# ChainSafe/lumenos

Measured on AMD Instinct MI355X. Metric: prove_eval_seconds_16384x4096, lower is better.
Workload: dtype u64; 1 GPU; Encode+Commit+InnerProduct(r,b)+QueryCols 16384x4096 LogN=14 L=12 K=2 rhoInv=2 queries=309; parallelism=1 GPU: the whole job resident in HBM

## Files before the change

### lumenos_amd/csrc/lm_keyswitch.hip

```cpp
#include <cstdlib>
#include <cstring>

#include "lm_ks_dev.h"

__host__ __device__ __forceinline__ size_t ks_ext_at(uint32_t b, uint32_t d, uint32_t t, uint32_t B, uint32_t beta) {
    return ((size_t)t * B + b) * beta + d;
}
__host__ __device__ __forceinline__ size_t ks_u_at(uint32_t pw, uint32_t t, uint32_t B, uint32_t L, uint32_t K) {
    return t < L ? (size_t)t * 2 * B + pw : (size_t)L * 2 * B + (size_t)pw * K + (t - L);
}
__host__ __device__ __forceinline__ size_t ks_key_at(uint32_t d, uint32_t w, uint32_t t, uint32_t beta) {
    return ((size_t)t * beta + d) * 2 + w;
}

static uint32_t ks_batch(const lumen_ctx *ctx) { return ctx->tune.ks_batch; }

__device__ __forceinline__ void mul128(u64 a, u64 b, u64 &lo, u64 &hi) {
    const u32 a0 = (u32)a, a1 = (u32)(a >> 32), b0 = (u32)b, b1 = (u32)(b >> 32);
    const u64 p0 = (u64)a0 * b0;
    const u64 p1 = lm_keep((u64)a0 * b1 + (p0 >> 32));
    const u64 p2 = lm_keep((u64)a1 * b0 + (u32)p1);
    hi = (u64)a1 * b1 + (p1 >> 32) + (p2 >> 32);
    lo = (p2 << 32) | (u32)p0;
}
// ... 42 lines not shown
            pack_pair(a, b, m0, m1, M, hi, lo);
            if (e) hv.y = hi, lv.y = lo;
            else hv.x = hi, lv.x = lo;
        }
        *reinterpret_cast<ulonglong2 *>(y0) = hv;
        *reinterpret_cast<ulonglong2 *>(y0 + N) = lv;
    }
}

template <int LOGN>
__global__ __launch_bounds__(lm_max_threads(LOGN)) void k_intt_pack(const u64 *__restrict__ acc, u64 *coef, uint32_t B,
                                                                  uint32_t L, uint32_t nf, lm_mods mods,
                                                                  lm_ninv_t yscale, const tw_t *__restrict__ tw_all) {
    extern __shared__ __attribute__((aligned(16))) u64 sm[];
    constexpr uint32_t N = 1u << LOGN;
    const uint32_t tid = threadIdx.x, nthreads = blockDim.x;
    if (blockIdx.x >= B * nf) {
        const uint32_t k = blockIdx.x - B * nf, l = 2 * nf + k / B, b = k % B;
        const u64 *p = acc + (((size_t)b * 2 + 1) * L + l) * N;
        u64 *o = coef + ((size_t)b * L + l) * N;
        const lm_qc q = lm_make_qc(mods.m[l]);
        const tw_t sc = yscale.t[l];
        auto ld = [&](uint32_t i0, u64 *v, int count) { lm_load_run(p, i0, v, count); };
        auto st = [&](uint32_t i, u64 v) { o[i] = lm_shoup_cs(v, sc, q.q, q.nq); };
        lm_ntt_inverse<LOGN>(sm, tw_all + (size_t)l * N, q, tid, nthreads, ld, st);
        return;
    }
    const uint32_t d = blockIdx.x / B, b = blockIdx.x % B;
    const uint32_t l0 = 2 * d, l1 = l0 + 1;
    const u64 *c1 = acc + ((size_t)b * 2 + 1) * L * N;
    u64 *o0 = coef + ((size_t)b * L + l0) * N;
    const lm_qc q0 = lm_make_qc(mods.m[l0]);
    const tw_t s0 = yscale.t[l0];
    {
        const u64 *p = c1 + (size_t)l0 * N;
        auto ld = [&](uint32_t i0, u64 *v, int count) { lm_load_run(p, i0, v, count); };
        auto st = [&](uint32_t i, u64 v) { o0[i] = lm_shoup_cs(v, s0, q0.q, q0.nq); };
        lm_ntt_inverse<LOGN>(sm, tw_all + (size_t)l0 * N, q0, tid, nthreads, ld, st);
    }
    __syncthreads();
    {
        const lm_qc q1 = lm_make_qc(mods.m[l1]);
        const tw_t s1 = yscale.t[l1];
        const u64 *p = c1 + (size_t)l1 * N;
        u64 Ml, Mh;
        mul128(q0.q, q1.q, Ml, Mh);
        auto uni = [](u64 x) {
            return (u64)(uint32_t)__builtin_amdgcn_readfirstlane((int)(uint32_t)x) |
                   (u64)(uint32_t)__builtin_amdgcn_readfirstlane((int)(uint32_t)(x >> 32)) << 32;
        };
        const u128 M = ((u128)uni(Mh) << 64) | uni(Ml);
        auto ld = [&](uint32_t i0, u64 *v, int count) { lm_load_run(p, i0, v, count); };
        constexpr int R_LAST = lm_pass_r(LOGN, 0), LOG_T0 = LOGN - R_LAST;
        constexpr int PF = (1 << R_LAST) * 5 / 8;
        struct pack_t {
            u64 *o0;
            const lm_qc &q0, &q1;
            tw_t s1;
            u128 M;
            u64 y0[PF];
            __device__ __forceinline__ void pre(uint32_t w) {
#pragma unroll
                for (int k = 0; k < PF; k++) y0[k] = o0[w + ((uint32_t)k << LOG_T0)];
            }
            __device__ __forceinline__ void operator()(uint32_t i, u64 v, int k) {
                const u64 y1 = lm_shoup_cs(v, s1, q1.q, q1.nq);
                uint32_t j = i;
                asm volatile("" : "+v"(j));
                const u64 a = k < PF ? y0[k < PF ? k : 0] : o0[j];
                u64 hi, lo;
                pack_pair(a, y1, q0.q, q1.q, M, hi, lo);
                o0[j] = hi, o0[j + N] = lo;
                if (k >= PF && (k & 1)) asm volatile("" ::: "memory");
            }
        } st{o0, q0, q1, s1, M, {}};
        uint32_t tid1 = tid;
        asm volatile("" : "+v"(tid1));
        lm_ntt_inverse<LOGN>(sm, tw_all + (size_t)l1 * N, q1, tid1, nthreads, ld, st);
    }
}

struct pt_consts_t {
    u64 c[LM_MAX_LIMBS];
};
__global__ void k_pt_prepare(const u64 *__restrict__ pt, u64 *__restrict__ ptM, uint32_t logN, uint32_t nl,
                             lm_mods mods, pt_consts_t pc) {
    const size_t total = (size_t)nl << logN;
    for (size_t i = (size_t)blockIdx.x * blockDim.x + threadIdx.x; i < total; i += (size_t)gridDim.x * blockDim.x) {
        const uint32_t limb = (uint32_t)(i >> logN);
        u64 lo, hi;
        mul128(pt[i], pc.c[limb], lo, hi);
        ptM[i] = lm_mont_reduce(lo, hi, mods.m[limb].q, mods.m[limb].qneg);
    }
}
__global__ void k_mul_plain(const u64 *__restrict__ ct, u64 *__restrict__ out, const u64 *__restrict__ ptM,
                            size_t words, uint32_t logN, uint32_t nl, lm_mods mods) {
    const size_t stride = (size_t)gridDim.x * blockDim.x;
    const size_t N = (size_t)1 << logN;
    for (size_t i = (size_t)blockIdx.x * blockDim.x + threadIdx.x; i < words; i += stride) {
        const uint32_t limb = (uint32_t)((i >> logN) % nl);
        const size_t k = i & (N - 1);
        u64 lo, hi;
        mul128(ct[i], ptM[(size_t)limb * N + k], lo, hi);
        out[i] = lm_mont_reduce(lo, hi, mods.m[limb].q, mods.m[limb].qneg);
    }
}

template <int LOGN>
__global__ __launch_bounds__(lm_fwdw_threads(LOGN), lm_fwdw_waves(LOGN)) void k_modup_ntt(const u64 *__restrict__ coef, const u64 *__restrict__ acc,
                                                    u64 *__restrict__ ext, const bx_t *__restrict__ bx,
                                                    uint32_t B, uint32_t L, uint32_t K, uint32_t beta,
                                                    const uint32_t *__restrict__ work, lm_mods mods,
                                                    const tw_t *__restrict__ tw_all) {
    extern __shared__ __attribute__((aligned(16))) u64 sm[];
    constexpr uint32_t N = 1u << LOGN;
    const uint32_t tid = threadIdx.x, nthreads = blockDim.x, LK = L + K;
    const uint32_t wk = work[blockIdx.x];
    const uint32_t b = wk & 0xFFFF, d = (wk >> 16) & 0xFF, t = wk >> 24;
    const bx_t c = bx[d * LK + t];
    u64 *o = ext + ks_ext_at(b, d, t, B, beta) * N;
    const lm_qc qc = lm_make_qc(mods.m[t]);
    const u64 *s0 = coef + ((size_t)b * L + d * K) * N;
    const u64 *s1 = c.ns == 2 ? s0 + N : s0;
    auto ld = [&](uint32_t i) { return bx_apply(c, s0[i], s1[i], qc); };
    auto out = [&](uint32_t j, u64 v0, u64 v1) {
        ulonglong2 y;
        y.x = v0, y.y = v1;
        *reinterpret_cast<ulonglong2 *>(o + j) = y;
    };
    if constexpr (LOGN == 14) {
        (void)nthreads;
        lm_w14_runs st{sm};
        auto after = [&](uint32_t i0, uint32_t) { lm_w14_linear_out(sm, tid, i0, out); };
        lm_ntt_forward_w14(sm, tw_all + (size_t)t * N, qc, tid, ld, st, after);
    } else {
        lm_lds_runs st{sm};
        auto after = [&](uint32_t, uint32_t) { lm_linear_out<LOGN>(sm, tid, out); };
        lm_ntt_forward<LOGN>(sm, tw_all + (size_t)t * N, qc, tid, nthreads, ld, st, after);
    }
}

#ifndef LM_MAC_COLS
#define LM_MAC_COLS 4
#endif
#ifndef LM_MAC_VEC
#define LM_MAC_VEC 1
#endif
#ifndef LM_MAC_PREFETCH
#define LM_MAC_PREFETCH 1
#endif
template <int VEC>
struct mac_vec;
template <>
struct mac_vec<1> {
    u64 v[1];
    static __device__ __forceinline__ mac_vec load(const u64 *p) { return mac_vec{{*p}}; }
    static __device__ __forceinline__ mac_vec load_once(const u64 *p) { return mac_vec{{__builtin_nontemporal_load(p)}}; }
    __device__ __forceinline__ void store(u64 *p) const { *p = v[0]; }
};
template <>
struct mac_vec<2> {
    u64 v[2];
    static __device__ __forceinline__ mac_vec load(const u64 *p) {
        const ulonglong2 a = *reinterpret_cast<const ulonglong2 *>(p);
        return mac_vec{{a.x, a.y}};
    }
    static __device__ __forceinline__ mac_vec load_once(const u64 *p) {
        return mac_vec{{__builtin_nontemporal_load(p), __builtin_nontemporal_load(p + 1)}};
    }
    __device__ __forceinline__ void store(u64 *p) const {
        ulonglong2 a;
        a.x = v[0], a.y = v[1];
        *reinterpret_cast<ulonglong2 *>(p) = a;
    }
};
struct mac_acc {
    u64 a0, a1, a3;
    u32 c0, c1;
    __device__ __forceinline__ void clear() { a0 = a1 = a3 = 0, c0 = c1 = 0; }
    __device__ __forceinline__ void value(u64 &lo, u64 &hi) const {
        lo = a0 + (a1 << 32);
        hi = a3 + c0 + (a1 >> 32) + ((u64)c1 << 32) + (lo < a0 ? 1 : 0);
    }
};
__device__ __forceinline__ void mac2(mac_acc &p, mac_acc &q, u64 x, u64 k0, u64 k1) {
    const u32 x0 = (u32)x, x1 = (u32)(x >> 32);
#if LM_ASM_SHOUP
    asm("v_mad_u64_u32 %[pa0], s[98:99], %[x0], %[k00], %[pa0]\n\t"
        "v_mad_u64_u32 %[qa0], s[90:91], %[x0], %[k10], %[qa0]\n\t"
        "v_mad_u64_u32 %[pa1], s[94:95], %[x0], %[k01], %[pa1]\n\t"
        "v_addc_co_u32_e64 %[pc0], s[96:97], %[pc0], 0, s[98:99]\n\t"
        "v_mad_u64_u32 %[qa1], s[92:93], %[x0], %[k11], %[qa1]\n\t"
        "v_addc_co_u32_e64 %[qc0], s[96:97], %[qc0], 0, s[90:91]\n\t"
        "v_mad_u64_u32 %[pa3], s[96:97], %[x1], %[k01], %[pa3]\n\t"
        "v_addc_co_u32_e64 %[pc1], s[96:97], %[pc1], 0, s[94:95]\n\t"
        "v_mad_u64_u32 %[pa1], s[98:99], %[x1], %[k00], %[pa1]\n\t"
        "v_addc_co_u32_e64 %[qc1], s[96:97], %[qc1], 0, s[92:93]\n\t"
        "v_mad_u64_u32 %[qa1], s[90:91], %[x1], %[k10], %[qa1]\n\t"
        "v_mad_u64_u32 %[qa3], s[96:97], %[x1], %[k11], %[qa3]\n\t"
        "v_addc_co_u32_e64 %[pc1], s[96:97], %[pc1], 0, s[98:99]\n\t"
        "v_addc_co_u32_e64 %[qc1], s[96:97], %[qc1], 0, s[90:91]"
        : [pa0] "+v"(p.a0), [pa1] "+v"(p.a1), [pa3] "+v"(p.a3), [pc0] "+v"(p.c0), [pc1] "+v"(p.c1),
          [qa0] "+v"(q.a0), [qa1] "+v"(q.a1), [qa3] "+v"(q.a3), [qc0] "+v"(q.c0), [qc1] "+v"(q.c1)
        : [x0] "v"(x0), [x1] "v"(x1), [k00] "v"((u32)k0), [k01] "v"((u32)(k0 >> 32)), [k10] "v"((u32)k1),
          [k11] "v"((u32)(k1 >> 32))
        : "s92", "s93", "s94", "s95", "s96", "s97", "s98", "s99", "s90", "s91");
#else
    auto one = [&](mac_acc &r, u64 k) {
        const u32 k0w = (u32)k, k1w = (u32)(k >> 32);
        u64 t = r.a0 + (u64)x0 * k0w;
        r.c0 += t < r.a0, r.a0 = t;
        t = r.a1 + (u64)x0 * k1w;
        r.c1 += t < r.a1, r.a1 = t;
        t = r.a1 + (u64)x1 * k0w;
        r.c1 += t < r.a1, r.a1 = t;
        r.a3 += (u64)x1 * k1w;
    };
    one(p, k0);
    one(q, k1);
#endif
}

__global__ __launch_bounds__(256) void k_ks_mac(const u64 *__restrict__ ext, const u64 *__restrict__ acc,
                                                const u64 *__restrict__ key, u64 *__restrict__ u, uint32_t B,
                                                uint32_t L, uint32_t K, uint32_t beta, uint32_t logN,
                                                lm_mods mods) {
    typedef mac_vec<LM_MAC_VEC> vec;
    const uint32_t N = 1u << logN, LK = L + K;
    const uint32_t G = (B + LM_MAC_COLS - 1) / LM_MAC_COLS, per_limb = N / (256 * LM_MAC_VEC) ? N / (256 * LM_MAC_VEC) : 1;
    const uint32_t slices = per_limb * LK;
    uint32_t slice, z;
    if (slices % 8 == 0) {
        const uint32_t xcd = blockIdx.x & 7, j = blockIdx.x >> 3;
        z = j % G;
        slice = (j / G) * 8 + xcd;
    } else {
        z = blockIdx.x % G;
        slice = blockIdx.x / G;
    }
    const uint32_t i = ((slice % per_limb) * 256 + threadIdx.x) * LM_MAC_VEC;
    const uint32_t t = LK - 1 - slice / per_limb;
    const uint32_t b0 = z * LM_MAC_COLS;
    if (i >= N) return;
    const mod_t md = mods.m[t];
    const uint32_t own = t < L ? t / K : 0xFFFFFFFFu;
    mac_acc a0[LM_MAC_COLS][LM_MAC_VEC], a1[LM_MAC_COLS][LM_MAC_VEC];
#pragma unroll
    for (int c = 0; c < LM_MAC_COLS; c++)
#pragma unroll
        for (int e = 0; e < LM_MAC_VEC; e++) a0[c][e].clear(), a1[c][e].clear();
    struct digit_t {
        vec k0, k1, x[LM_MAC_COLS];
    };
    auto fetch = [&](uint32_t d) {
        digit_t g;
        g.k0 = vec::load(key + ks_key_at(d, 0, t, beta) * N + i);
        g.k1 = vec::load(key + ks_key_at(d, 1, t, beta) * N + i);
#pragma unroll
        for (int c = 0; c < LM_MAC_COLS; c++) {
            const uint32_t bc = b0 + c < B ? b0 + c : B - 1;
            g.x[c] = d == own ? vec::load(acc + ((size_t)(bc * 2 + 1) * L + t) * N + i)
                              : vec::load_once(ext + ks_ext_at(bc, d, t, B, beta) * N + i);
        }
        return g;
    };
    constexpr int PF = LM_MAC_PREFETCH;
    digit_t q[PF + 1];
#pragma unroll
    for (int j = 0; j < PF; j++)
        if ((uint32_t)j < beta) q[j] = fetch(j);
    for (uint32_t d0 = 0; d0 < beta; d0 += PF + 1) {
#pragma unroll
        for (int j = 0; j <= PF; j++) {
            const uint32_t d = d0 + j;
            if (d < beta) {
                if (d + PF < beta) q[(j + PF) % (PF + 1)] = fetch(d + PF);
#pragma unroll
                for (int c = 0; c < LM_MAC_COLS; c++)
#pragma unroll
                    for (int e = 0; e < LM_MAC_VEC; e++) mac2(a0[c][e], a1[c][e], q[j].x[c].v[e], q[j].k0.v[e], q[j].k1.v[e]);
            }
        }
    }
#pragma unroll
    for (int c = 0; c < LM_MAC_COLS; c++) {
        if (b0 + c < B) {
            u64 *o = u + ks_u_at((b0 + c) * 2, t, B, L, K) * N + i, *o1 = u + ks_u_at((b0 + c) * 2 + 1, t, B, L, K) * N + i;
            vec r0, r1;
#pragma unroll
            for (int e = 0; e < LM_MAC_VEC; e++) {
                u64 lo, hi;
                a0[c][e].value(lo, hi);
                r0.v[e] = lm_mont_reduce_wide(lo, hi, md.q, md.qneg, md.qinv64, beta);
                a1[c][e].value(lo, hi);
                r1.v[e] = lm_mont_reduce_wide(lo, hi, md.q, md.qneg, md.qinv64, beta);
            }
            r0.store(o);
            r1.store(o1);
        }
    }
}

template <int LOGN>
__global__ __launch_bounds__(lm_max_threads(LOGN)) void k_moddown_ntt(const u64 *__restrict__ u, const u64 *__restrict__ acc_in,
                                                     u64 *__restrict__ acc_out, const bx_t *__restrict__ bxp,
                                                     const tw_t *__restrict__ pinv,
                                                     const uint32_t *__restrict__ index,
                                                     const uint32_t *__restrict__ inv_index,
                                                     const uint32_t *__restrict__ work, uint32_t B,
                                                     uint32_t L, uint32_t K, lm_mods mods,
                                                     const tw_t *__restrict__ tw_all) {
    extern __shared__ __attribute__((aligned(16))) u64 sm[];
    constexpr uint32_t N = 1u << LOGN;
    const uint32_t tid = threadIdx.x, nthreads = blockDim.x;
    const uint32_t wk = work[blockIdx.x];
    const uint32_t pw = wk & 0xFFFF;
    const uint32_t t = wk >> 16;
    const uint32_t w = pw & 1;
    const bx_t c = bxp[t];
    const lm_qc qc = lm_make_qc(mods.m[t]);
    const u64 *up0 = u + ks_u_at(pw, L, B, L, K) * N;
    const u64 *up1 = c.ns == 2 ? up0 + N : up0;
    const u64 *uq = u + ks_u_at(pw, t, B, L, K) * N;
    const u64 *ain = acc_in + ((size_t)pw * L + t) * N;
    u64 *aout = acc_out + ((size_t)pw * L + t) * N;
    tw_t pi = pinv[t];
    pi.w = qc.q - pi.w, pi.wp = ~pi.wp;
    auto ld = [&](uint32_t i) { return bx_apply(c, up0[i], up1[i], qc); };
    constexpr int RUN = lm_fwd_run<LOGN>();
    static_assert(RUN <= 8, "lm_load_run moves at most 8 coefficients");
    struct storer_t {
        const u64 *uq, *ain;
        u64 *sm;
        const lm_qc &qc;
        tw_t pi;
        uint32_t w;
        u64 uv[RUN], cv[RUN];
        __device__ __forceinline__ void pre(uint32_t i0) {
            lm_load_run(uq, i0, uv, RUN);
            if (w == 0) lm_load_run(ain, i0, cv, RUN);
        }
        __device__ __forceinline__ void operator()(uint32_t i0, const u64 *v, int count) {
#pragma unroll
            for (int k = 0; k < RUN; k++)
                if (k < count) {
                    const u64 add = w == 0 ? uv[k] + cv[k] : uv[k];
                    sm[LM_PAD(i0 + k)] = lm_shoup3<true>(v[k], pi.w, pi.wp, qc.nq, add);
                }
        }
    } st{uq, ain, sm, qc, pi, w, {}, {}};
    constexpr uint32_t NW = lm_nthreads(LOGN) / 64, BLK = N / NW, IT = BLK / 128;
    const uint32_t wave = tid >> 6, lane = tid & 63;
    const uint32_t jb = NW > 1 ? (uint32_t)__builtin_amdgcn_readfirstlane((int)(inv_index[wave * BLK] / BLK)) : 0u;
    auto after = [&](uint32_t, uint32_t) {
        uint2 p[IT];
        ulonglong2 x[IT];
#pragma unroll
        for (uint32_t k = 0; k < IT; k++) {
            const uint32_t j = jb * BLK + 2 * lane + k * 128;
            p[k] = *reinterpret_cast<const uint2 *>(index + j);
            x[k] = *reinterpret_cast<const ulonglong2 *>(ain + j);
        }
        lm_wave_sync();
#pragma unroll
        for (uint32_t k = 0; k < IT; k++) {
            const uint32_t j = jb * BLK + 2 * lane + k * 128;
            ulonglong2 y;
            y.x = lm_csub(lm_csub(x[k].x + sm[LM_PAD(p[k].x)], 4 * qc.q), 2 * qc.q);
            y.y = lm_csub(lm_csub(x[k].y + sm[LM_PAD(p[k].y)], 4 * qc.q), 2 * qc.q);
            *reinterpret_cast<ulonglong2 *>(aout + j) = y;
        }
    };
    lm_ntt_forward<LOGN>(sm, tw_all + (size_t)t * N, qc, tid, nthreads, ld, st, after);
}

__global__ __launch_bounds__(256) void k_acc_canon(u64 *__restrict__ acc, size_t pairs, uint32_t logN, uint32_t L, lm_mods mods) {
    const size_t stride = (size_t)gridDim.x * blockDim.x;
    for (size_t g = (size_t)blockIdx.x * blockDim.x + threadIdx.x; g < pairs; g += stride) {
        const u64 q = mods.m[(uint32_t)((g >> (logN - 1)) % L)].q;
        ulonglong2 v = *reinterpret_cast<ulonglong2 *>(acc + 2 * g);
        v.x = lm_csub(v.x, q), v.y = lm_csub(v.y, q);
        *reinterpret_cast<ulonglong2 *>(acc + 2 * g) = v;
    }
}

namespace {

int acc_canon(lumen_ctx *ctx, u64 *acc, size_t words, uint32_t L) {
    if (!words) return 0;
    hipLaunchKernelGGL(k_acc_canon, dim3(2048), dim3(256), 0, ctx->stream, acc, words / 2, ctx->logN, L, ctx->mods);
    LM_HIP(ctx, hipGetLastError());
    return 0;
}

struct KsTables {
    bx_t *d_bx = nullptr;
    bx_t *d_bxp = nullptr;
    tw_t *d_pinv = nullptr;
    uint32_t beta = 0;
    lm_ninv_t yscale;
    std::vector<uint16_t> pairs;
    std::map<uint32_t, uint32_t *> d_work;
    std::map<uint32_t, uint32_t *> d_work_down;
    ~KsTables() {
        for (auto &kv : d_work) hipFree(kv.second);
        for (auto &kv : d_work_down) hipFree(kv.second);
        hipFree(d_bx);
        hipFree(d_bxp);
        hipFree(d_pinv);
    }
};

bx_t make_bx(const uint64_t *src, uint32_t ns, uint64_t t) {
    bx_t c;
    memset(&c, 0, sizeof(c));
    c.ns = ns;
    uint64_t m_mod_t = 1;
    for (uint32_t a = 0; a < ns; a++) m_mod_t = h_mulmod(m_mod_t, src[a] % t, t);
    c.b57 = h_tw((1ull << LM_W_SPLIT) % t, t);
    c.c_t = (t - h_mulmod(2 % t, m_mod_t, t)) % t;
    return c;
}

uint64_t hat_inv(const uint64_t *src, uint32_t ns, uint32_t a) {
    uint64_t h = 1;
    for (uint32_t b = 0; b < ns; b++)
        if (b != a) h = h_mulmod(h, src[b] % src[a], src[a]);
    return h_invmod(h, src[a]);
}

int get_tables(lumen_ctx *ctx, KsTables **out) {
    LM_SHARED_LOCK(ctx);
    auto it = ctx->ext.find("ks_tables");
    if (it != ctx->ext.end()) {
        *out = static_cast<KsTables *>(it->second.get());
        return 0;
    }
    const uint32_t L = ctx->L, K = ctx->K, LK = L + K;
    LM_CHECK(ctx, K >= 1 && K <= 2, "key switching supports 1 or 2 special primes (have %u)", K);
    auto sp = std::make_shared<KsTables>();
    KsTables &tb = *sp;
    tb.beta = (L + K - 1) / K;
    std::vector<bx_t> bx((size_t)tb.beta * LK);
    for (uint32_t d = 0; d < tb.beta; d++) {
        const uint32_t lo = d * K, hi = std::min(lo + K, L), ns = hi - lo;
        for (uint32_t t = 0; t < LK; t++) {
            bx_t c = make_bx(ctx->mod + lo, ns, ctx->mod[t]);
            c.own = (t >= lo && t < hi) ? 1 : 0;
            bx[(size_t)d * LK + t] = c;
        }
    }
    for (uint32_t i = 0; i < LM_MAX_LIMBS; i++) tb.yscale.t[i] = ctx->ninv[i < LK ? i : 0];
    for (uint32_t d = 0; d < tb.beta; d++) {
        const uint32_t lo = d * K, hi = std::min(lo + K, L), ns = hi - lo;
        for (uint32_t a = 0; a < ns; a++) {
            const uint64_t m = ctx->mod[lo + a];
            tb.yscale.t[lo + a] = h_tw(h_mulmod(ctx->ninv[lo + a].w, hat_inv(ctx->mod + lo, ns, a), m), m);
        }
    }
    for (uint32_t a = 0; a < K; a++) {
        const uint64_t m = ctx->mod[L + a];
        tb.yscale.t[L + a] = h_tw(h_mulmod(ctx->ninv[L + a].w, hat_inv(ctx->mod + L, K, a), m), m);
    }
    std::vector<bx_t> bxp(L);
    std::vector<tw_t> pinv(L);
    for (uint32_t t = 0; t < L; t++) {
        bxp[t] = make_bx(ctx->mod + L, K, ctx->mod[t]);
        uint64_t q = ctx->mod[t], P = 1;
        for (uint32_t a = 0; a < K; a++) P = h_mulmod(P, ctx->mod[L + a] % q, q);
        pinv[t] = h_tw(h_invmod(P, q), q);
    }
    std::vector<uint16_t> pairs;
    for (uint32_t t = 0; t < LK; t++)
        for (uint32_t d = 0; d < tb.beta; d++)
            if (!bx[(size_t)d * LK + t].own) pairs.push_back((uint16_t)(d | (t << 8)));
    tb.pairs = pairs;
    LM_HIP(ctx, hipMalloc((void **)&tb.d_bx, bx.size() * sizeof(bx_t)));
    LM_HIP(ctx, hipMalloc((void **)&tb.d_bxp, bxp.size() * sizeof(bx_t)));
    LM_HIP(ctx, hipMalloc((void **)&tb.d_pinv, pinv.size() * sizeof(tw_t)));
    LM_HIP(ctx, hipMemcpy(tb.d_bx, bx.data(), bx.size() * sizeof(bx_t), hipMemcpyHostToDevice));
    LM_HIP(ctx, hipMemcpy(tb.d_bxp, bxp.data(), bxp.size() * sizeof(bx_t), hipMemcpyHostToDevice));
    LM_HIP(ctx, hipMemcpy(tb.d_pinv, pinv.data(), pinv.size() * sizeof(tw_t), hipMemcpyHostToDevice));
    ctx->ext["ks_tables"] = sp;
    *out = sp.get();
    return 0;
}

}

int lm_ks_tables_view(lumen_ctx *ctx, lm_ks_view *out) {
    KsTables *tb = nullptr;
    if (int rc = get_tables(ctx, &tb)) return rc;
    out->d_bxp = tb->d_bxp;
    out->d_pinv = tb->d_pinv;
    out->yscale = &tb->yscale;
    return 0;
}

int lm_launch_pack_v(lumen_ctx *ctx, u64 *y, size_t poly_stride, uint32_t npoly, uint32_t ngroups,
                     uint32_t group_limbs, uint32_t first_mod, uint32_t nlimbs_total) {
    hipLaunchKernelGGL(k_pack_v, dim3(2048), dim3(256), 0, ctx->stream, y, poly_stride, npoly, ngroups, group_limbs,
                       first_mod, nlimbs_total, ctx->logN, ctx->mods);
    LM_HIP(ctx, hipGetLastError());
    return 0;
}

namespace {

struct KsScratch {
    u64 *coef, *ext, *u, *acc2;
};

static int modup_work_list(lumen_ctx *ctx, KsTables *tb, uint32_t B, const uint32_t **out) {
    const uint32_t LM_MODUP_TGROUP = ctx->tune.modup_tgroup;
    LM_SHARED_LOCK(ctx);
    LM_CHECK(ctx, B >= 1 && B <= 65535 && tb->beta <= 255 && ctx->L + ctx->K <= 255,
             "key-switch batch of %u columns (beta %u) does not fit the packed work list", B, tb->beta);
    const uint32_t cache_key = B | (LM_MODUP_TGROUP << 16);
    auto it = tb->d_work.find(cache_key);
    if (it != tb->d_work.end()) {
        *out = it->second;
        return 0;
    }
    const uint32_t LK = ctx->L + ctx->K, beta = tb->beta;
    std::vector<std::vector<uint8_t>> need(beta);
    for (uint16_t pr : tb->pairs) need[pr & 0xFF].push_back((uint8_t)(pr >> 8));
    std::vector<std::vector<uint32_t>> lists(8);
    for (uint32_t x = 0; x < 8; x++)
        for (uint32_t t0 = 0; t0 < LK; t0 += LM_MODUP_TGROUP)
            for (uint32_t b = x; b < B; b += 8)
                for (uint32_t d = 0; d < beta; d++)
                    for (uint8_t t : need[d])
                        if (t >= t0 && t < t0 + LM_MODUP_TGROUP) lists[x].push_back(b | (d << 16) | ((uint32_t)t << 24));
    std::vector<uint32_t> order;
    order.reserve((size_t)B * tb->pairs.size());
    std::vector<size_t> pos(8, 0);
    for (bool any = true; any;) {
        any = false;
        for (uint32_t x = 0; x < 8; x++)
            if (pos[x] < lists[x].size()) {
                order.push_back(lists[x][pos[x]++]);
                any = true;
            }
    }
    LM_CHECK(ctx, order.size() == (size_t)B * tb->pairs.size(), "extension work list is inconsistent");
    uint32_t *d = nullptr;
    LM_HIP(ctx, hipMalloc((void **)&d, order.size() * sizeof(uint32_t)));
    LM_HIP(ctx, hipMemcpy(d, order.data(), order.size() * sizeof(uint32_t), hipMemcpyHostToDevice));
    tb->d_work[cache_key] = d;
    *out = d;
    return 0;
}

static int moddown_work_list(lumen_ctx *ctx, KsTables *tb, uint32_t B, const uint32_t **out) {
    const uint32_t LM_MODDOWN_TGROUP = ctx->tune.moddown_tgroup;
    LM_SHARED_LOCK(ctx);
    LM_CHECK(ctx, B >= 1 && 2 * (uint64_t)B <= 65535, "key-switch batch of %u columns does not fit the packed work list", B);
    const uint32_t cache_key = B | (LM_MODDOWN_TGROUP << 17);
    auto it = tb->d_work_down.find(cache_key);
    if (it != tb->d_work_down.end()) {
        *out = it->second;
        return 0;
    }
    const uint32_t L = ctx->L;
    std::vector<std::vector<uint32_t>> lists(8);
    for (uint32_t x = 0; x < 8; x++)
        for (uint32_t t0 = 0; t0 < L; t0 += LM_MODDOWN_TGROUP)
            for (uint32_t pw = x; pw < 2 * B; pw += 8)
                for (uint32_t t = t0; t < std::min<uint32_t>(t0 + LM_MODDOWN_TGROUP, L); t++) lists[x].push_back(pw | (t << 16));
    std::vector<uint32_t> order;
    order.reserve((size_t)2 * B * L);
    std::vector<size_t> pos(8, 0);
    for (bool any = true; any;) {
        any = false;
        for (uint32_t x = 0; x < 8; x++)
            if (pos[x] < lists[x].size()) {
                order.push_back(lists[x][pos[x]++]);
                any = true;
            }
    }
    LM_CHECK(ctx, order.size() == (size_t)2 * B * L, "ModDown work list is inconsistent");
    uint32_t *d = nullptr;
    LM_HIP(ctx, hipMalloc((void **)&d, order.size() * sizeof(uint32_t)));
    LM_HIP(ctx, hipMemcpy(d, order.data(), order.size() * sizeof(uint32_t), hipMemcpyHostToDevice));
    tb->d_work_down[cache_key] = d;
    *out = d;
    return 0;
}

static uint32_t ks_lanes(const lumen_ctx *ctx) {
    return ctx->tune.ks_lanes ? ctx->tune.ks_lanes : (ctx->logN <= 13 ? 2 : 1);
}
template <int LOGN>
static uint32_t intt_pack_slots(lumen_ctx *ctx) {
    static const uint32_t v = [&] {
        hipDeviceProp_t prop;
        int per_cu = 0;
        if (hipGetDeviceProperties(&prop, ctx->device) != hipSuccess) return 256u;
        (void)hipFuncSetAttribute(reinterpret_cast<const void *>(&k_intt_pack<LOGN>),
                                  hipFuncAttributeMaxDynamicSharedMemorySize, 160 * 1024);
        if (hipOccupancyMaxActiveBlocksPerMultiprocessor(&per_cu, k_intt_pack<LOGN>, lm_nthreads(LOGN),
                                                         lm_lds_for(1u << LOGN)) != hipSuccess || per_cu < 1) {
            per_cu = (int)std::max<size_t>(1, std::min<size_t>(160 * 1024 / lm_lds_for(1u << LOGN), 2048 / lm_nthreads(LOGN)));
        }
        (void)hipGetLastError();
        if (ctx->tune.debug)
            fprintf(stderr, "[lumenos_hip] k_intt_pack<%d>: %d workgroup(s) per CU, %d CUs\n", LOGN, per_cu,
                    prop.multiProcessorCount);
        return (uint32_t)prop.multiProcessorCount * (uint32_t)per_cu;
    }();
    return v;
}
static uint32_t ks_fused_digits(lumen_ctx *ctx, uint32_t B, uint32_t L) {
    const long forced = ctx->tune.ks_fused_digits;
    const uint32_t pairs = L / 2;
    if (forced >= 0) return std::min<uint32_t>((uint32_t)forced, pairs);
    uint32_t slots = 0;
    switch (ctx->logN) {
#define LM_CASE(n) \
    case n: slots = intt_pack_slots<n>(ctx); break;
        LM_FOR_EACH_LOGN(LM_CASE)
#undef LM_CASE
    default: return 0;
    }
    for (uint32_t nf = pairs; nf >= 1; nf--)
        if (((uint64_t)B * nf) % slots == 0) return nf;
    return 0;
}

struct LaneGuard {
    lumen_ctx *ctx;
    hipStream_t saved;
    LaneGuard(lumen_ctx *c, int lane) : ctx(c), saved(c->stream) {
        if (lane) ctx->stream = ctx->stream2;
    }
    ~LaneGuard() { ctx->stream = saved; }
};

int rotate_accumulate(lumen_ctx *ctx, const u64 *acc, u64 *acc_out, uint32_t B, const lm_galois_key &gk,
                      KsTables *tb, const KsScratch &s) {
    const uint32_t N = ctx->N, L = ctx->L, K = ctx->K, LK = L + K, beta = tb->beta;
    const size_t lds = lm_fwd_lds(ctx->logN);
    const uint32_t threads = lm_fwd_threads(ctx->logN);
    const uint32_t nf = K == 2 ? ks_fused_digits(ctx, B, L) : 0;
    if (nf) {
        const size_t lds_i = lm_inv_lds(ctx->logN);
        const uint32_t grid = B * nf + B * (L - 2 * nf);
        lm_prof_scope ps(ctx, "ks_intt_c1", (uint64_t)B * L);
        switch (ctx->logN) {
#define LM_CASE(n)                                                                                              \
    case n:                                                                                                     \
        LM_LDS_ATTR(ctx, k_intt_pack<n>, lds_i);                                                                \
        hipLaunchKernelGGL(k_intt_pack<n>, dim3(grid), dim3(lm_inv_threads(ctx->logN)), lds_i, ctx->stream, acc, \
                           s.coef, B, L, nf, ctx->mods, tb->yscale, ctx->d_tw_inv);                             \
        break;
            LM_FOR_EACH_LOGN(LM_CASE)
#undef LM_CASE
        default:
            return lm_fail(ctx, "ring degree 2^%u has no kernel instantiation", ctx->logN);
        }
        LM_HIP(ctx, hipGetLastError());
    } else {
        if (int rc = lm_launch_ntt_strided(ctx, acc + (size_t)L * N, (size_t)2 * L * N, s.coef, (size_t)L * N, B,
                                           lm_map_q(L), true, "ks_intt_c1", &tb->yscale))
            return rc;
    }
    if (K == 2 && nf < beta) {
        lm_prof_scope ps(ctx, "ks_pack_v", (uint64_t)B);
        hipLaunchKernelGGL(k_pack_v, dim3(2048), dim3(256), 0, ctx->stream, s.coef + (size_t)2 * nf * N, (size_t)L * N,
                           B, beta - nf, K, 2 * nf, L - 2 * nf, ctx->logN, ctx->mods);
        LM_HIP(ctx, hipGetLastError());
    }
    {
        const uint64_t nb = (uint64_t)B * tb->pairs.size();
        const uint32_t *work = nullptr;
        if (int rc = modup_work_list(ctx, tb, B, &work)) return rc;
        lm_prof_scope ps(ctx, "ks_modup_ntt", nb);
        const lm_geom gm = lm_fwdw_geom(ctx->logN);
        switch (ctx->logN) {
#define LM_CASE(n)                                                                                            \
    case n:                                                                                                   \
        LM_LDS_ATTR(ctx, k_modup_ntt<n>, gm.lds);                                                             \
        hipLaunchKernelGGL(k_modup_ntt<n>, dim3((uint32_t)nb), dim3(gm.threads), gm.lds, ctx->stream, s.coef, acc, \
                           s.ext, tb->d_bx, B, L, K, beta, work, ctx->mods, ctx->d_tw_fwd);                   \
        break;
            LM_FOR_EACH_LOGN(LM_CASE)
#undef LM_CASE
        default:
            return lm_fail(ctx, "ring degree 2^%u has no kernel instantiation", ctx->logN);
        }
        LM_HIP(ctx, hipGetLastError());
    }
    {
        lm_prof_scope ps(ctx, "ks_mac", (uint64_t)B);
        dim3 grid(((N / LM_MAC_VEC + 255) / 256) * LK * ((B + LM_MAC_COLS - 1) / LM_MAC_COLS));
        hipLaunchKernelGGL(k_ks_mac, grid, dim3(256), 0, ctx->stream, s.ext, acc, gk.d_key, s.u, B, L, K, beta,
                           ctx->logN, ctx->mods);
        LM_HIP(ctx, hipGetLastError());
    }
    {
        lm_modmap mp;
        mp.period = K;
        for (uint32_t i = 0; i < LM_MAX_LIMBS; i++) mp.idx[i] = (uint8_t)(L + (i < K ? i : 0));
        u64 *up = s.u + ks_u_at(0, L, B, L, K) * N;
        const size_t pstride = (size_t)K * N;
        if (int rc = lm_launch_ntt_strided(ctx, up, pstride, up, pstride, B * 2, mp, true, "ks_intt_p", &tb->yscale))
            return rc;
        if (K == 2) {
            lm_prof_scope ps(ctx, "ks_pack_v", (uint64_t)B);
            hipLaunchKernelGGL(k_pack_v, dim3(2048), dim3(256), 0, ctx->stream, up, pstride, B * 2, 1u, K, L, K,
                               ctx->logN, ctx->mods);
            LM_HIP(ctx, hipGetLastError());
        }
    }
    {
        const uint32_t *work_down = nullptr;
        if (int rc = moddown_work_list(ctx, tb, B, &work_down)) return rc;
        lm_prof_scope ps(ctx, "ks_moddown_ntt", (uint64_t)B * 2 * L);
        switch (ctx->logN) {
#define LM_CASE(n)                                                                                            \
    case n:                                                                                                   \
        LM_LDS_ATTR(ctx, k_moddown_ntt<n>, lds);               \
        hipLaunchKernelGGL(k_moddown_ntt<n>, dim3(B * 2 * L), dim3(threads), lds, ctx->stream, s.u, acc,      \
                           acc_out, tb->d_bxp, tb->d_pinv, gk.d_index, gk.d_inv_index, work_down, B, L, K, ctx->mods, \
                           ctx->d_tw_fwd);                                                                    \
        break;
            LM_FOR_EACH_LOGN(LM_CASE)
#undef LM_CASE
        default:
            return lm_fail(ctx, "ring degree 2^%u has no kernel instantiation", ctx->logN);
        }
        LM_HIP(ctx, hipGetLastError());
    }
    return 0;
}

int get_scratch(lumen_ctx *ctx, uint32_t B, KsTables *tb, KsScratch *s, int lane = 0, u64 **group_acc = nullptr,
                size_t group_acc_bytes = 0) {
    const size_t N = ctx->N, L = ctx->L, LK = ctx->L + ctx->K, beta = tb->beta;
    const char *names[2][5] = {{"ks_coef", "ks_ext", "ks_u", "ks_acc2", "ks_acc"}, {"ks_coef_b", "ks_ext_b", "ks_u_b", "ks_acc2_b", "ks_acc"}};
    const int NB = group_acc ? 5 : 4;
    const size_t bytes[5] = {(size_t)B * L * N * 8, (size_t)B * beta * LK * N * 8, (size_t)B * 2 * LK * N * 8, (size_t)B * 2 * L * N * 8,
                             std::max(group_acc_bytes, (size_t)B * 2 * L * N * 8)};
    u64 *dummy = nullptr;
    u64 **slot[5] = {&s->coef, &s->ext, &s->u, &s->acc2, group_acc ? group_acc : &dummy};
    bool have = true;
    for (int c = 0; c < NB; c++) {
        auto it = ctx->scratch.find(names[lane][c]);
        have = have && it != ctx->scratch.end() && it->second.first && it->second.second >= bytes[c];
    }
    lm_galois_key gk;
    {
        LM_SHARED_LOCK(ctx);
        if (!ctx->gkeys.empty()) gk = ctx->gkeys.begin()->second;
    }
    const uint32_t Kc = ctx->tune.ks_placement;
    auto plain = [&]() -> int {
        bool ok = true;
        for (int c = 0; c < NB; c++) ok = (*slot[c] = (u64 *)lm_scratch(ctx, names[lane][c], bytes[c])) != nullptr && ok;
        return ok ? 0 : 1;
    };
    if (have || Kc < 2 || bytes[1] < ((size_t)64 << 20) || !gk.d_key) return plain();
    std::vector<void *> cand[5];
    bool fixed[5] = {false, false, false, false, false};
    for (int c = 0; c < NB; c++) {
        auto it = ctx->scratch.find(names[lane][c]);
        if (it != ctx->scratch.end() && it->second.first && it->second.second >= bytes[c]) cand[c].push_back(it->second.first), fixed[c] = true;
    }
    void *probe_acc = nullptr;
    auto free_all = [&] {
        for (int c = 0; c < NB; c++)
            if (!fixed[c])
                for (void *p : cand[c]) hipFree(p);
        hipFree(probe_acc);
        (void)hipGetLastError();
    };
    size_t free_b = 0, total_b = 0, drawn = 0;
    (void)hipMemGetInfo(&free_b, &total_b);
    if (!group_acc && hipMalloc(&probe_acc, bytes[3]) != hipSuccess) probe_acc = nullptr;
    for (uint32_t k = 0; k < Kc; k++)
        for (int c = 0; c < NB; c++) {
            if (fixed[c] || (c == 4 && k >= 4)) continue;
            if (!cand[c].empty() && drawn + bytes[c] > free_b / 2) continue;
            void *p = nullptr;
            if (hipMalloc(&p, bytes[c]) == hipSuccess) cand[c].push_back(p), drawn += bytes[c];
        }
    (void)hipGetLastError();
    bool complete = group_acc || probe_acc;
    for (int c = 0; c < NB; c++) complete = complete && !cand[c].empty();
    if (!complete) {
        free_all();
        return plain();
    }
    const bool prof = ctx->prof;
    ctx->prof = false;
    hipEvent_t e0 = lm_ev_get(ctx), e1 = lm_ev_get(ctx);
    size_t pick[5] = {0, 0, 0, 0, 0};
    int rc = 0;
    auto eval = [&](float *ms) -> int {
        KsScratch t;
        t.coef = (u64 *)cand[0][pick[0]], t.ext = (u64 *)cand[1][pick[1]], t.u = (u64 *)cand[2][pick[2]], t.acc2 = (u64 *)cand[3][pick[3]];
        u64 *a0 = group_acc ? (u64 *)cand[4][pick[4]] : (u64 *)probe_acc;
        u64 *a1 = group_acc ? a0 + (bytes[4] - bytes[3]) / 8 : a0;
        for (int r = 0; r < 3; r++) {
            if (r == 1) LM_HIP(ctx, hipEventRecord(e0, ctx->stream));
            u64 *a = r == 2 ? a1 : a0;
            if (int e = rotate_accumulate(ctx, a, t.acc2, B, gk, tb, t)) return e;
            if (int e = rotate_accumulate(ctx, t.acc2, a, B, gk, tb, t)) return e;
        }
        LM_HIP(ctx, hipEventRecord(e1, ctx->stream));
        LM_HIP(ctx, hipEventSynchronize(e1));
        LM_HIP(ctx, hipEventElapsedTime(ms, e0, e1));
        return 0;
    };
    float first = 0, best_all = 0;
    static const int order[5] = {2, 1, 4, 3, 0};
    bool measured = false;
    for (int oi = 0; oi < 5 && !rc; oi++) {
        const int c = order[oi];
        if (c >= NB) continue;
        float best = 0;
        size_t arg = pick[c];
        for (size_t k = 0; k < cand[c].size() && !rc; k++) {
            if (measured && k == pick[c]) continue;
            const size_t keep = pick[c];
            pick[c] = k;
            float ms = 0;
            rc = eval(&ms);
            pick[c] = keep;
            if (first == 0) first = ms;
            if (best == 0 || ms < best) best = ms, arg = k;
        }
        if (best == 0 || (measured && best_all <= best)) arg = pick[c];
        else best_all = best;
        if (best != 0) measured = true;
        pick[c] = arg;
    }
    ctx->ev_pool.push_back(e0);
    ctx->ev_pool.push_back(e1);
    ctx->prof = prof;
    if (rc) {
        lm_sync_all(ctx);
        free_all();
        return rc;
    }
    if (ctx->tune.debug)
        fprintf(stderr, "[lumenos_hip] key-switch scratch placement (lane %d, %u columns): %zu / %zu / %zu candidates for u / ext / the group "
                        "accumulator, 4 rotations of the first draw %.3f ms, of the chosen blocks %.3f ms\n", lane, B, cand[2].size(),
                cand[1].size(), NB == 5 ? cand[4].size() : (size_t)0, first, best_all);
    LM_HIP(ctx, hipStreamSynchronize(ctx->stream));
    for (int c = 0; c < NB; c++) {
        void *chosen = cand[c][pick[c]];
        if (!fixed[c]) {
            cand[c][pick[c]] = nullptr;
            lm_scratch_adopt(ctx, names[lane][c], chosen, bytes[c]);
        }
        *slot[c] = (u64 *)chosen;
    }
    free_all();
    return 0;
}

int inner_sum_batch(lumen_ctx *ctx, u64 *acc, uint32_t B, uint32_t n, KsTables *tb, const KsScratch &s) {
    uint64_t gal[64];
    const uint32_t cnt = lumen_inner_sum_galois_elements(ctx, n, gal);
    for (uint32_t r = 0; r < cnt; r++) {
        lm_galois_key gk;
        {
            LM_SHARED_LOCK(ctx);
            auto it = ctx->gkeys.find(gal[r]);
            LM_CHECK(ctx, it != ctx->gkeys.end(), "Galois key for element %llu not loaded",
                     (unsigned long long)gal[r]);
            gk = it->second;
        }
        u64 *src = (r & 1) ? s.acc2 : acc, *dst = (r & 1) ? acc : s.acc2;
        if (int rc = rotate_accumulate(ctx, src, dst, B, gk, tb, s)) return rc;
    }
    if (cnt & 1)
        LM_HIP(ctx, hipMemcpyAsync(acc, s.acc2, (size_t)B * 2 * ctx->L * ctx->N * 8, hipMemcpyDeviceToDevice,
                                   ctx->stream));
    return 0;
}

int upload_ptT(lumen_ctx *ctx, const uint64_t *pt, uint32_t nl, u64 **out) {
    const uint32_t N = ctx->N;
    const size_t words = (size_t)nl * N;
    u64 *h = (u64 *)lm_stage(ctx, words * sizeof(u64));
    u64 *draw = (u64 *)lm_scratch(ctx, "pt_raw", words * sizeof(u64));
    u64 *d = (u64 *)lm_scratch(ctx, "ptT", words * sizeof(u64));
    if (!h || !draw || !d) return 1;
    pt_consts_t pc;
    memset(&pc, 0, sizeof(pc));
    for (uint32_t l = 0; l < nl; l++) {
        const uint64_t q = ctx->mod[l];
        const uint64_t *src = pt + (size_t)l * N;
        uint64_t bad = 0;
        for (uint32_t k = 0; k < N; k++) bad |= (uint64_t)(src[k] >= q);
        if (bad) return lm_fail(ctx, "plaintext residue out of range at limb %u", l);
        memcpy(h + (size_t)l * N, src, (size_t)N * sizeof(u64));
        const uint64_t r = (uint64_t)((((u128)1) << 64) % q);
        pc.c[l] = h_mulmod(ctx->T % q, h_mulmod(r, r, q), q);
    }
    LM_HIP(ctx, hipMemcpyAsync(draw, h, words * sizeof(u64), hipMemcpyHostToDevice, ctx->stream));
    LM_HIP(ctx, hipEventRecord(ctx->ev_stage, ctx->stream));
    hipLaunchKernelGGL(k_pt_prepare, dim3(256), dim3(256), 0, ctx->stream, draw, d, ctx->logN, nl, ctx->mods, pc);
    LM_HIP(ctx, hipGetLastError());
    *out = d;
    return 0;
}

int launch_mul_plain(lumen_ctx *ctx, const u64 *ct, u64 *out, const u64 *ptT, size_t words, uint32_t nl,
                     uint32_t ncts) {
    lm_prof_scope ps(ctx, "mul_plain", ncts);
    hipLaunchKernelGGL(k_mul_plain, dim3(4096), dim3(256), 0, ctx->stream, ct, out, ptT, words, ctx->logN, nl,
                       ctx->mods);
    LM_HIP(ctx, hipGetLastError());
    ctx->mul_counter += ncts;
    return 0;
}

}

extern "C" int lumen_ks_mac_probe(lumen_ctx *ctx, uint32_t batch, const void *ext, const void *acc, const void *key,
                                  void *u, uint32_t reps, float *ms_per_launch) {
    LM_CHECK(nullptr, ctx && ms_per_launch, "lumen_ks_mac_probe: NULL argument");
    LM_ENTER(ctx);
    KsTables *tb = nullptr;
    if (int rc = get_tables(ctx, &tb)) return rc;
    const uint32_t N = ctx->N, L = ctx->L, K = ctx->K, LK = L + K, B = batch ? batch : ks_batch(ctx);
    LM_CHECK(ctx, B <= 65535 && reps >= 1 && reps <= 100000, "lumen_ks_mac_probe: batch %u / reps %u out of range", B, reps);
    KsScratch s;
    if (int rc = get_scratch(ctx, B, tb, &s)) return rc;
    if (!acc) acc = lm_scratch(ctx, "ks_acc", (size_t)B * 2 * L * N * 8);
    if (!acc) return 1;
    if (!key) {
        LM_SHARED_LOCK(ctx);
        LM_CHECK(ctx, !ctx->gkeys.empty(), "lumen_ks_mac_probe: no Galois key loaded");
        key = ctx->gkeys.begin()->second.d_key;
    }
    const u64 *pe = ext ? (const u64 *)ext : s.ext;
    u64 *pu = u ? (u64 *)u : s.u;
    dim3 grid(((N / LM_MAC_VEC + 255) / 256) * LK * ((B + LM_MAC_COLS - 1) / LM_MAC_COLS));
    auto launch = [&] {
        hipLaunchKernelGGL(k_ks_mac, grid, dim3(256), 0, ctx->stream, pe, (const u64 *)acc, (const u64 *)key, pu, B, L, K,
                           tb->beta, ctx->logN, ctx->mods);
    };
    for (int i = 0; i < 3; i++) launch();
    LM_HIP(ctx, hipGetLastError());
    LM_HIP(ctx, hipEventRecord(ctx->tm0, ctx->stream));
    for (uint32_t i = 0; i < reps; i++) launch();
    LM_HIP(ctx, hipGetLastError());
    LM_HIP(ctx, hipEventRecord(ctx->tm1, ctx->stream));
    LM_HIP(ctx, hipEventSynchronize(ctx->tm1));
    float ms = 0;
    LM_HIP(ctx, hipEventElapsedTime(&ms, ctx->tm0, ctx->tm1));
    *ms_per_launch = ms / (float)reps;
    return 0;
}

extern "C" uint32_t lumen_inner_sum_galois_elements(const lumen_ctx *ctx, uint32_t n, uint64_t *gal_els) {
    if (!ctx || !gal_els || n == 0 || (n & (n - 1))) return 0;
    const uint64_t two_n = 2ull * ctx->N;
    const uint32_t span = n == ctx->N ? n >> 1 : n;
    uint32_t cnt = 0;
    uint64_t g = 5;
    for (uint32_t r = 1; r < span; r <<= 1) {
        gal_els[cnt++] = g;
        g = (g * g) & (two_n - 1);
    }
    if (n == ctx->N) gal_els[cnt++] = two_n - 1;
    return cnt;
}

__global__ __launch_bounds__(256) void k_key_prepare(const u64 *__restrict__ src, u64 *__restrict__ dst, uint32_t logN, uint32_t LK,
                                                     size_t words, lm_mods mods, lm_ninv_t fac, uint32_t *__restrict__ bad) {
    const uint32_t beta = (uint32_t)((words >> logN) / (2 * LK));
    for (size_t i = (size_t)blockIdx.x * blockDim.x + threadIdx.x; i < words; i += (size_t)gridDim.x * blockDim.x) {
        const uint32_t row = (uint32_t)(i >> logN), t = row % LK;
        const u64 q = mods.m[t].q, x = src[i];
        if (x >= q) atomicMin(bad, row);
        const size_t o = (ks_key_at(row / (2 * LK), (row / LK) & 1, t, beta) << logN) + (i & (((size_t)1 << logN) - 1));
        dst[o] = lm_shoup_cs(x, fac.t[t], q, 0 - q);
    }
}

int lm_h2d(lumen_ctx *ctx, void *dev, const void *host, size_t bytes);

extern "C" int lumen_load_galois_key_ex(lumen_ctx *ctx, uint64_t gal_el, const uint64_t *evk, uint32_t flags) {
    LM_CHECK(nullptr, ctx && evk, "lumen_load_galois_key: NULL argument");
    LM_ENTER(ctx);
    const uint32_t N = ctx->N, L = ctx->L, K = ctx->K, LK = L + K;
    LM_CHECK(ctx, K >= 1, "parameters have no special primes: key switching unavailable");
    LM_CHECK(ctx, (gal_el & 1) && gal_el < 2ull * N, "Galois element %llu is not an odd residue mod 2N",
             (unsigned long long)gal_el);
    LM_CHECK(ctx, !(flags & ~(uint32_t)LUMEN_KEY_MONTGOMERY), "lumen_load_galois_key_ex: unknown flags 0x%x", flags);
    const uint32_t beta = (L + K - 1) / K;
    const size_t words = (size_t)beta * 2 * LK * N;
    lm_ninv_t fac;
    for (uint32_t t = 0; t < LM_MAX_LIMBS; t++) fac.t[t] = h_tw(1, ctx->mod[0] ? ctx->mod[0] : 3);
    for (uint32_t t = 0; t < LK; t++) {
        const uint64_t q = ctx->mod[t];
        uint64_t r = (flags & LUMEN_KEY_MONTGOMERY) ? 1 : (uint64_t)((((u128)1) << 64) % q);
        if (t < L) {
            uint64_t P = 1;
            for (uint32_t a = 0; a < K; a++) P = h_mulmod(P, ctx->mod[L + a] % q, q);
            r = h_mulmod(r, h_invmod(P, q), q);
        }
        fac.t[t] = h_tw(r, q);
    }
    u64 *raw = (u64 *)lm_scratch(ctx, "key_raw", words * 8);
    uint32_t *bad = (uint32_t *)lm_scratch(ctx, "key_bad", 4);
    if (!raw || !bad) return 1;
    LM_HIP(ctx, hipMemsetAsync(bad, 0xFF, 4, ctx->stream));
    if (int rc = lm_h2d(ctx, raw, evk, words * 8)) return rc;
    u64 *d_new = nullptr;
    LM_HIP(ctx, hipMalloc((void **)&d_new, words * 8));
    hipLaunchKernelGGL(k_key_prepare, dim3(2048), dim3(256), 0, ctx->stream, raw, d_new, ctx->logN, LK, words, ctx->mods, fac, bad);
    uint32_t first_bad = 0;
    hipError_t e = hipGetLastError();
    if (e == hipSuccess) e = hipMemcpyAsync(&first_bad, bad, 4, hipMemcpyDeviceToHost, ctx->stream);
    if (e == hipSuccess) e = hipStreamSynchronize(ctx->stream);
    if (e != hipSuccess || first_bad != 0xFFFFFFFFu) {
        hipFree(d_new);
        if (e != hipSuccess) return lm_fail(ctx, "key conversion failed: %s", hipGetErrorString(e));
        return lm_fail(ctx, "key residue out of range (digit %u limb %u)", first_bad / (2 * LK), first_bad % LK);
    }
// ... 141 lines not shown
```

Before: 1.748 s.

## Specialize moddown NTT for LogN=14 with wave-level forward NTT and deferred c0 add

For ring degree 2^14 the moddown kernel now uses a dedicated wave-oriented forward NTT (lm_ntt_forward_w14) with its own LDS position mapping. Each wave serves two 1024-element output blocks instead of one. The c0 accumulator add moves out of the storer into a post-NTT sweep over LDS, and some uq loads are issued late to cut register pressure. The launch geometry and bounds come from new fwdw helpers with a minimum-waves hint, trading code complexity for better occupancy and less early-load pressure.

```diff
diff --git a/lumenos_amd/csrc/lm_keyswitch.hip b/lumenos_amd/csrc/lm_keyswitch.hip
--- a/lumenos_amd/csrc/lm_keyswitch.hip
+++ b/lumenos_amd/csrc/lm_keyswitch.hip
@@ -368,7 +368,7 @@
 }
 
 template <int LOGN>
-__global__ __launch_bounds__(lm_max_threads(LOGN)) void k_moddown_ntt(const u64 *__restrict__ u, const u64 *__restrict__ acc_in,
+__global__ __launch_bounds__(lm_fwdw_threads(LOGN), lm_fwdw_waves(LOGN)) void k_moddown_ntt(const u64 *__restrict__ u, const u64 *__restrict__ acc_in,
                                                      u64 *__restrict__ acc_out, const bx_t *__restrict__ bxp,
                                                      const tw_t *__restrict__ pinv,
                                                      const uint32_t *__restrict__ index,
@@ -394,6 +394,7 @@
     pi.w = qc.q - pi.w, pi.wp = ~pi.wp;
     auto ld = [&](uint32_t i) { return bx_apply(c, up0[i], up1[i], qc); };
     constexpr int RUN = lm_fwd_run<LOGN>();
+    constexpr bool C0_IN_PRE = LOGN != 14;
     static_assert(RUN <= 8, "lm_load_run moves at most 8 coefficients");
     struct storer_t {
         const u64 *uq, *ain;
@@ -402,42 +403,72 @@
         tw_t pi;
         uint32_t w;
         u64 uv[RUN], cv[RUN];
+        static __device__ __forceinline__ bool late(uint32_t i0) { return LOGN == 14 && (i0 & (3u << 9)) == 0; }
         __device__ __forceinline__ void pre(uint32_t i0) {
-            lm_load_run(uq, i0, uv, RUN);
-            if (w == 0) lm_load_run(ain, i0, cv, RUN);
+            if (!late(i0)) lm_load_run(uq, i0, uv, RUN);
+            if (C0_IN_PRE && w == 0) lm_load_run(ain, i0, cv, RUN);
         }
         __device__ __forceinline__ void operator()(uint32_t i0, const u64 *v, int count) {
+            if (late(i0)) {
+                __builtin_amdgcn_sched_barrier(0);
+                lm_load_run(uq, i0, uv, RUN);
+            }
 #pragma unroll
             for (int k = 0; k < RUN; k++)
                 if (k < count) {
-                    const u64 add = w == 0 ? uv[k] + cv[k] : uv[k];
-                    sm[LM_PAD(i0 + k)] = lm_shoup3<true>(v[k], pi.w, pi.wp, qc.nq, add);
+                    const u64 add = C0_IN_PRE && w == 0 ? uv[k] + cv[k] : uv[k];
+                    sm[LOGN == 14 ? lm_w14_pos(i0) + k : LM_PAD(i0 + k)] = lm_shoup3<true>(v[k], pi.w, pi.wp, qc.nq, add);
                 }
         }
     } st{uq, ain, sm, qc, pi, w, {}, {}};
-    constexpr uint32_t NW = lm_nthreads(LOGN) / 64, BLK = N / NW, IT = BLK / 128;
+    constexpr uint32_t BLK = LOGN == 14 ? 1024u : N / (lm_nthreads(LOGN) / 64), NB = N / BLK, IT = BLK / 128;
     const uint32_t wave = tid >> 6, lane = tid & 63;
-    const uint32_t jb = NW > 1 ? (uint32_t)__builtin_amdgcn_readfirstlane((int)(inv_index[wave * BLK] / BLK)) : 0u;
-    auto after = [&](uint32_t, uint32_t) {
+    auto serve = [&](uint32_t jb, auto pos) {
         uint2 p[IT];
         ulonglong2 x[IT];
+        const uint32_t l2 = 2 * lane;
 #pragma unroll
         for (uint32_t k = 0; k < IT; k++) {
-            const uint32_t j = jb * BLK + 2 * lane + k * 128;
+            const uint32_t j = jb * BLK + l2 + k * 128;
             p[k] = *reinterpret_cast<const uint2 *>(index + j);
             x[k] = *reinterpret_cast<const ulonglong2 *>(ain + j);
         }
         lm_wave_sync();
 #pragma unroll
         for (uint32_t k = 0; k < IT; k++) {
-            const uint32_t j = jb * BLK + 2 * lane + k * 128;
+            const uint32_t j = jb * BLK + l2 + k * 128;
             ulonglong2 y;
-            y.x = lm_csub(lm_csub(x[k].x + sm[LM_PAD(p[k].x)], 4 * qc.q), 2 * qc.q);
-            y.y = lm_csub(lm_csub(x[k].y + sm[LM_PAD(p[k].y)], 4 * qc.q), 2 * qc.q);
+            y.x = lm_csub(lm_csub(x[k].x + sm[pos(p[k].x)], 4 * qc.q), 2 * qc.q);
+            y.y = lm_csub(lm_csub(x[k].y + sm[pos(p[k].y)], 4 * qc.q), 2 * qc.q);
             *reinterpret_cast<ulonglong2 *>(aout + j) = y;
         }
     };
-    lm_ntt_forward<LOGN>(sm, tw_all + (size_t)t * N, qc, tid, nthreads, ld, st, after);
+    auto jb_of = [&](uint32_t src) {
+        return NB > 1 ? (uint32_t)__builtin_amdgcn_readfirstlane((int)(inv_index[src * BLK] / BLK)) : 0u;
+    };
+    if constexpr (LOGN == 14) {
+        (void)nthreads;
+        const uint32_t jb0 = jb_of(2 * wave), jb1 = jb_of(2 * wave + 1);
+        auto c0_sweep = [&](uint32_t i0) {
+            const uint32_t l2 = 2 * lane, base = (wave << 11) | i0;
+#pragma unroll
+            for (uint32_t k = 0; k < IT; k++) {
+                const uint32_t j = base | (l2 + k * 128);
+                const ulonglong2 cv = *reinterpret_cast<const ulonglong2 *>(ain + j);
+                const uint32_t pj = lm_w14_pos(j);
+                sm[pj] += cv.x, sm[pj + 1] += cv.y;
+            }
+        };
+        auto after = [&](uint32_t i0, uint32_t) {
+            if (w == 0) c0_sweep(i0);
+            serve(i0 ? jb1 : jb0, [](uint32_t i) { return lm_w14_pos(i); });
+        };
+        lm_ntt_forward_w14(sm, tw_all + (size_t)t * N, qc, tid, ld, st, after);
+    } else {
+        const uint32_t jb = jb_of(wave);
+        auto after = [&](uint32_t, uint32_t) { serve(jb, [](uint32_t i) { return (uint32_t)LM_PAD(i); }); };
+        lm_ntt_forward<LOGN>(sm, tw_all + (size_t)t * N, qc, tid, nthreads, ld, st, after);
+    }
 }
 
 __global__ __launch_bounds__(256) void k_acc_canon(u64 *__restrict__ acc, size_t pairs, uint32_t logN, uint32_t L, lm_mods mods) {
@@ -706,8 +737,6 @@
 int rotate_accumulate(lumen_ctx *ctx, const u64 *acc, u64 *acc_out, uint32_t B, const lm_galois_key &gk,
                       KsTables *tb, const KsScratch &s) {
     const uint32_t N = ctx->N, L = ctx->L, K = ctx->K, LK = L + K, beta = tb->beta;
-    const size_t lds = lm_fwd_lds(ctx->logN);
-    const uint32_t threads = lm_fwd_threads(ctx->logN);
     const uint32_t nf = K == 2 ? ks_fused_digits(ctx, B, L) : 0;
     if (nf) {
         const size_t lds_i = lm_inv_lds(ctx->logN);
@@ -783,11 +812,12 @@
         const uint32_t *work_down = nullptr;
         if (int rc = moddown_work_list(ctx, tb, B, &work_down)) return rc;
         lm_prof_scope ps(ctx, "ks_moddown_ntt", (uint64_t)B * 2 * L);
+        const lm_geom gm = lm_fwdw_geom(ctx->logN);
         switch (ctx->logN) {
 #define LM_CASE(n)                                                                                            \
     case n:                                                                                                   \
-        LM_LDS_ATTR(ctx, k_moddown_ntt<n>, lds);               \
-        hipLaunchKernelGGL(k_moddown_ntt<n>, dim3(B * 2 * L), dim3(threads), lds, ctx->stream, s.u, acc,      \
+        LM_LDS_ATTR(ctx, k_moddown_ntt<n>, gm.lds);                                                           \
+        hipLaunchKernelGGL(k_moddown_ntt<n>, dim3(B * 2 * L), dim3(gm.threads), gm.lds, ctx->stream, s.u, acc, \
                            acc_out, tb->d_bxp, tb->d_pinv, gk.d_index, gk.d_inv_index, work_down, B, L, K, ctx->mods, \
                            ctx->d_tw_fwd);                                                                    \
         break;
```

Result: no change. 1.734 s, median of 6 (-0.8%).
